# CRIMAC-WP4-Machine-learning/CRIMAC-classifiers-unet

Measured on AMD Instinct MI355X. Metric: echogram patches/sec (4ch 256x256), training step (fwd+weighted CE+bwd+SGD), higher is better.
Workload: dtype bf16; 1 GPU; BASELINE configs[1]: U-Net (depth 5, 64 filters) train step, batch 32 x 4x256x256 per GPU; global_batch=32, precision=bf16, start_filts=64, parallelism=dp1, ranks=1, launcher=single process

## Files before the change

crimac_classifiers_unet_amd/csrc/elementwise.hip:

```cpp
#include <stdarg.h>
#include <stdlib.h>

#include <mutex>

#include "common.h"
#include "bnb_sums.h"

static thread_local char g_err[512] = "";
void crimac_set_error(const char* fmt, ...) {
  va_list ap;
  va_start(ap, fmt);
  vsnprintf(g_err, sizeof(g_err), fmt, ap);
  va_end(ap);
}
extern "C" const char* crimac_last_error(void) { return g_err; }
extern "C" int crimac_version(void) { return CRIMAC_ABI_VERSION; }
extern "C" int crimac_layer_desc_size(void) { return (int)sizeof(crimac_layer_desc); }

namespace {

#ifdef CRIMAC_STREAM_FORWARD
#define CRIMAC_ROW(x, M) (x)
#else
#define CRIMAC_ROW(x, M) ((M) - 1 - (x))
#endif

constexpr int kMaxBlocks = 2048;

inline int grid_for(long work_items, int per_block) {
  long b = (work_items + per_block - 1) / per_block;
  if (b < 1) b = 1;
  if (b > kMaxBlocks) b = kMaxBlocks;
  return (int)b;
}

struct ResidentEntry { const void* fn; int dev, blocks; };
static ResidentEntry g_resident[96];
static int g_resident_n = 0;
static std::mutex g_resident_mu;
template <typename K>
inline int whole_rounds(K kernel, size_t lds, int grid, int block = 256) {
  int dev = 0;
  if (grid <= 256 || hipGetDevice(&dev) != hipSuccess) return grid;
  const void* fn = reinterpret_cast<const void*>(kernel);
  int blocks = 0;
  {
    std::lock_guard<std::mutex> lk(g_resident_mu);
    for (int i = 0; i < g_resident_n; ++i)
      if (g_resident[i].fn == fn && g_resident[i].dev == dev) blocks = g_resident[i].blocks;
    if (blocks == 0) {
      int per_cu = 0, cus = 0;
      if (hipOccupancyMaxActiveBlocksPerMultiprocessor(&per_cu, kernel, block, lds) == hipSuccess &&
          hipDeviceGetAttribute(&cus, hipDeviceAttributeMultiprocessorCount, dev) == hipSuccess && per_cu > 0 && cus > 0)
        blocks = per_cu * cus;
      else
        blocks = -1;
      if (g_resident_n < 96) g_resident[g_resident_n++] = ResidentEntry{fn, dev, blocks};
    }
  }
  return (blocks > 0 && grid > blocks) ? blocks : grid;
}

template <typename T>
__global__ void nchw_to_nhwc_kernel(const float* __restrict__ in, T* __restrict__ out, int C, long HW,
                                    long npix, long ld) {
  for (long p = blockIdx.x * (long)blockDim.x + threadIdx.x; p < npix;
       p += (long)gridDim.x * blockDim.x) {
    long b, hw;
    pix_split(p, HW, b, hw);
    const float* src = in + b * C * HW + hw;
    T* dst = out + p * ld;
    for (int c0 = 0; c0 < ld; c0 += 8) {
      float v[8];
#pragma unroll
      for (int j = 0; j < 8; ++j) v[j] = (c0 + j) < C ? src[(long)(c0 + j) * HW] : 0.f;
      store8(dst + c0, v);
// ... 73 lines not shown
      const float v = w[((long)ci * Co + co) * 4 + ab] * pf.fwd_scale;
      if (pf.interleaved) put_planes_il(v, pf.fwd_fp16, fwd_hi, r, ci, Ci);
      else put_planes(v, pf.npl, pf.fwd_fp16, fwd_hi, fwd_lo, i, n);
    }
    if (dg_hi) {
      const int co = (int)(i % Co);
      const long r = i / Co;
      const int ci = (int)(r % Ci), ab = (int)(r / Ci);
      const float v = w[((long)ci * Co + co) * 4 + ab] * pf.dg_scale;
      if (pf.interleaved) put_planes_il(v, pf.dg_fp16, dg_hi, r, co, Co);
      else put_planes(v, pf.npl, pf.dg_fp16, dg_hi, dg_lo, i, n);
    }
  }
}

__global__ void unpack_wgrad_conv_kernel(const float* __restrict__ dw, int Co, int Ci, int Ci_pad,
                                         float* __restrict__ grad) {
  const long n = (long)Co * Ci * 9;
  for (long i = blockIdx.x * (long)blockDim.x + threadIdx.x; i < n;
       i += (long)gridDim.x * blockDim.x) {
    const int t = (int)(i % 9);
    const long r = i / 9;
    const int ci = (int)(r % Ci), co = (int)(r / Ci);
    grad[i] = dw[((long)t * Co + co) * Ci_pad + ci];
  }
}

__global__ void unpack_wgrad_upconv_kernel(const float* __restrict__ dw, int Ci, int Co,
                                           float* __restrict__ grad) {
  const long n = (long)Ci * Co * 4;
  for (long i = blockIdx.x * (long)blockDim.x + threadIdx.x; i < n;
       i += (long)gridDim.x * blockDim.x) {
    const int ab = (int)(i % 4);
    const long r = i / 4;
    const int co = (int)(r % Co), ci = (int)(r / Co);
    grad[i] = dw[((long)ab * Ci + ci) * Co + co];
  }
}

template <typename T, typename ACC, int NQ, int UNR = 2, typename OP>
__device__ __forceinline__ void colreduce(long M, int C, OP op, ACC* out0, ACC* out1) {
  extern __shared__ __attribute__((aligned(16))) unsigned char smem_raw[];
  float* lds = reinterpret_cast<float*>(smem_raw);
  const int cpr = C / 8;
  const int rpi = 256 / cpr > 0 ? 256 / cpr : 1;
  for (int i = threadIdx.x; i < NQ * C; i += 256) lds[i] = 0.f;
  __syncthreads();
  const int chunk = threadIdx.x % cpr, rl = threadIdx.x / cpr;
  float s0[8], s1[8];
#pragma unroll
  for (int j = 0; j < 8; ++j) { s0[j] = 0.f; s1[j] = 0.f; }
// ... 1066 lines not shown

extern "C" int crimac_pack_upconv2x2(const float* w, int Ci, int Co, int planes, void* fwd_hi,
                                     void* fwd_lo, void* dg_hi, void* dg_lo, void* stream) {
  CRIMAC_REQUIRE(w && fwd_hi && Co > 0 && Ci > 0, "pack_upconv2x2: bad arguments");
  CRIMAC_REQUIRE(planes_arg_ok(planes) && ((planes & 15) == 1 || (planes & CRIMAC_PLANES_INTERLEAVED) || fwd_lo) &&
                     ((planes & 15) == 1 || (planes & CRIMAC_PLANES_INTERLEAVED) || !dg_hi || dg_lo),
                 "pack_upconv2x2: planes=%d needs the lo plane buffers", planes);
  const int grid = grid_for(4L * Co * Ci, 256);
  hipLaunchKernelGGL(pack_upconv_kernel, dim3(grid), dim3(256), 0, ST, w, Ci, Co, planes,
                     (unsigned short*)fwd_hi, (unsigned short*)fwd_lo, (unsigned short*)dg_hi,
                     (unsigned short*)dg_lo);
  CRIMAC_LAUNCH_CHECK();
  return CRIMAC_OK;
}

extern "C" int crimac_unpack_wgrad_conv3x3(const float* dw, int Co, int Ci, int Ci_pad, float* grad,
                                           void* stream) {
  CRIMAC_REQUIRE(dw && grad && Co > 0 && Ci > 0 && Ci_pad >= Ci, "unpack_wgrad_conv3x3: bad arguments");
  hipLaunchKernelGGL(unpack_wgrad_conv_kernel, dim3(grid_for(9L * Co * Ci, 256)), dim3(256), 0, ST, dw,
                     Co, Ci, Ci_pad, grad);
  CRIMAC_LAUNCH_CHECK();
  return CRIMAC_OK;
}

extern "C" int crimac_unpack_wgrad_upconv2x2(const float* dw, int Ci, int Co, float* grad,
                                             void* stream) {
  CRIMAC_REQUIRE(dw && grad && Co > 0 && Ci > 0, "unpack_wgrad_upconv2x2: bad arguments");
  hipLaunchKernelGGL(unpack_wgrad_upconv_kernel, dim3(grid_for(4L * Co * Ci, 256)), dim3(256), 0, ST,
                     dw, Ci, Co, grad);
  CRIMAC_LAUNCH_CHECK();
  return CRIMAC_OK;
}

static int colreduce_grid(long M, int C) {
  const int cpr = C / 8;
  const int rpi = 256 / cpr > 0 ? 256 / cpr : 1;
  return grid_for(M, rpi * 16);
}

extern "C" int crimac_colstats(int prec, const void* y, long ld, long M, int C, double* sum,
                               double* sumsq, void* stream) {
  PREC_OK("colstats");
  CRIMAC_REQUIRE(y && sum && M > 0 && C > 0 && C % 8 == 0 && C <= 2048 && ld >= C && ld % 8 == 0,
                 "colstats: bad arguments (C=%d ld=%ld)", C, ld);
  const int grid = colreduce_grid(M, C);
  const size_t lds = 2 * C * sizeof(float);
// ... 408 lines not shown
```

crimac_classifiers_unet_amd/csrc/pack.hip:

```cpp
#include "common.h"

namespace {

constexpr int kMaxLayers = 32;
constexpr int TILE = 32;

struct LayerDesc {
  const float* w;
  float* grad;
  const float* dw;
  unsigned short* fwd_hi;
  unsigned short* fwd_lo;
  unsigned short* dg_hi;
  unsigned short* dg_lo;
  int kind, Co, Ci, Ci_pad;
  int dw_splits;
  long dw_stride;
  int frag;
};

struct Table {
  LayerDesc d[kMaxLayers];
  int first[kMaxLayers + 1];
  int n;
// ... 46 lines not shown
    *reinterpret_cast<u32x4*>((k == 0 ? hi : lo + (long)(k - 1) * n) + i) = w;
  }
}

__device__ __forceinline__ void put_planes8_il(float (&v)[8], unsigned short* buf, long row, int col, int rowlen, int fp16) {
  unsigned short* dst = buf + row * 2L * rowlen + il_pos(col, rowlen);
  put_planes8(v, 2, dst, dst + il_cb(rowlen), 0, 0, fp16);
}

__device__ __forceinline__ void put_planes8_il_frag(float (&v)[8], unsigned short* buf, int t, int r, int R, int col, int rowlen,
                                                    int fp16) {
  const int c = (int)il_pos(col, rowlen);
  unsigned short* hi = buf + wfrag_index(t, r, c, R, 2 * rowlen);
  unsigned short* lo = buf + wfrag_index(t, r, c + il_cb(rowlen), R, 2 * rowlen);
  put_planes8(v, 2, hi, lo, 0, 0, fp16);
}

__global__ __launch_bounds__(256) void pack_layers_kernel(Table tb, int planes_arg) {
  __shared__ float tile[TILE][TILE * 9 + 1];
  const PlaneFmt pf = plane_fmt(planes_arg);
  const int npl = pf.npl;
  const int l = find_layer(tb, blockIdx.x);
  const LayerDesc& d = tb.d[l];
  const Geo g = geo_of(d.kind, d.Co, d.Ci, d.Ci_pad);
  const int tidx = blockIdx.x - tb.first[l];
  const int o0 = (tidx / g.tiles_inner) * TILE, i0 = (tidx % g.tiles_inner) * TILE;
  const int T = g.taps, run = TILE * T;
  const int valid = (g.inner - i0 < TILE ? (g.inner - i0 > 0 ? g.inner - i0 : 0) : TILE) * T;
  for (int ol = threadIdx.x >> 6; ol < TILE; ol += 4) {
    const float* src = d.w + ((long)(o0 + ol) * g.inner + i0) * T;
// ... 67 lines not shown
  float* base = tb.dw[l] + 4L * i;
  const long st = tb.stride[l];
  f32x4 acc = *reinterpret_cast<const f32x4*>(base + j * st);
  int k = j + kFold;
  for (; k + 3 * kFold < tb.splits[l]; k += 4 * kFold) {
    const f32x4 a = *reinterpret_cast<const f32x4*>(base + (long)k * st);
    const f32x4 b = *reinterpret_cast<const f32x4*>(base + (long)(k + kFold) * st);
    const f32x4 c = *reinterpret_cast<const f32x4*>(base + (long)(k + 2 * kFold) * st);
    const f32x4 d = *reinterpret_cast<const f32x4*>(base + (long)(k + 3 * kFold) * st);
    acc += a; acc += b; acc += c; acc += d;
  }
  for (; k < tb.splits[l]; k += kFold) acc += *reinterpret_cast<const f32x4*>(base + (long)k * st);
  *reinterpret_cast<f32x4*>(base + j * st) = acc;
}

__global__ __launch_bounds__(256) void unpack_layers_kernel(Table tb) {
  __shared__ float tile[TILE][TILE * 9 + 1];
  const int l = find_layer(tb, blockIdx.x);
  const LayerDesc& d = tb.d[l];
  const Geo g = geo_of(d.kind, d.Co, d.Ci, d.Ci_pad);
  const int tidx = blockIdx.x - tb.first[l];
  const int o0 = (tidx / g.tiles_inner) * TILE, i0 = (tidx % g.tiles_inner) * TILE;
  const int T = g.taps, run = TILE * T;
  const int nin = g.inner - i0 < TILE ? (g.inner - i0 > 0 ? g.inner - i0 : 0) : TILE;
#pragma unroll 2
  for (int idx = threadIdx.x; idx < T * TILE * TILE; idx += 256) {
    const int il = idx % TILE, ol = (idx / TILE) % TILE, t = idx / (TILE * TILE);
    if (il < nin) {
      const float* src = d.dw + ((long)t * g.outer + o0 + ol) * g.inner_pad + i0 + il;
      const int nsl = d.dw_splits < kFold ? d.dw_splits : kFold;
      float v0 = src[0], v1 = 0.f, v2 = 0.f, v3 = 0.f;
      int sp = 1;
      for (; sp + 3 < nsl; sp += 4) {
        const float a = src[(long)sp * d.dw_stride], b = src[(long)(sp + 1) * d.dw_stride];
        const float c = src[(long)(sp + 2) * d.dw_stride], e = src[(long)(sp + 3) * d.dw_stride];
        v0 += a; v1 += b; v2 += c; v3 += e;
      }
      for (; sp < nsl; ++sp) v0 += src[(long)sp * d.dw_stride];
      tile[ol][il * T + t] = (v0 + v1) + (v2 + v3);
    }
  }
  __syncthreads();
  const int valid = nin * T;
  for (int ol = threadIdx.x >> 6; ol < TILE; ol += 4) {
    float* dst = d.grad + ((long)(o0 + ol) * g.inner + i0) * T;
    for (int r = threadIdx.x & 63; r < valid; r += 64) dst[r] = tile[ol][r];
  }
}

struct HostDesc {
  const float* w;
  float* grad;
  const float* dw;
  void *fwd_hi, *fwd_lo, *dg_hi, *dg_lo;
  int kind, Co, Ci, Ci_pad;
  int dw_splits;
  long dw_stride;
};

int run_layers(const HostDesc* descs, int n, int mode, int planes_arg, hipStream_t st) {
  const int planes = planes_arg & 15;
  for (int base = 0; base < n; base += kMaxLayers) {
    Table tb;
    tb.n = n - base < kMaxLayers ? n - base : kMaxLayers;
    int total = 0;
    for (int i = 0; i < tb.n; ++i) {
      HostDesc h = descs[base + i];
      const int frag = ((h.kind & CRIMAC_LAYER_FWD_FRAG) ? 1 : 0) | ((h.kind & CRIMAC_LAYER_DG_FRAG) ? 2 : 0);
      CRIMAC_REQUIRE((h.kind & ~(3 | CRIMAC_LAYER_FWD_FRAG | CRIMAC_LAYER_DG_FRAG)) == 0 && (h.kind & 3) != 3 && h.Co > 0 &&
                     h.Ci > 0, "layer %d: bad kind/shape", base + i);
      h.kind &= 3;
      if (frag && mode == 0) {
        const bool ilv = (planes_arg & CRIMAC_PLANES_INTERLEAVED) != 0;
        const int kq = ilv ? 32 : 64;
        CRIMAC_REQUIRE(h.kind == 0 && (planes == 1 || ilv),
                       "layer %d: fragment-major planes are a single-plane 16-bit or interleaved-pair Conv2d layout", base + i);
        CRIMAC_REQUIRE(!(frag & 1) || (h.Co % 32 == 0 && h.Ci_pad % kq == 0), "layer %d: fragment-major forward plane needs "
                       "Co %% 32 == 0 and Ci_pad %% %d == 0 (Co=%d Ci_pad=%d)", base + i, kq, h.Co, h.Ci_pad);
        CRIMAC_REQUIRE(!(frag & 2) || (h.dg_hi && h.Ci % 32 == 0 && h.Co % kq == 0 && h.Ci_pad == h.Ci),
                       "layer %d: fragment-major input-gradient plane needs Ci %% 32 == 0 and Co %% %d == 0", base + i, kq);
      }
      CRIMAC_REQUIRE(h.Co % TILE == 0 && (h.kind == 0 || h.Ci % TILE == 0),
                     "layer %d: Co (and the transposed convolution's Ci) must be multiples of %d", base + i, TILE);
      CRIMAC_REQUIRE(h.kind == 1 || (h.Ci_pad >= h.Ci && h.Ci_pad % 2 == 0), "layer %d: bad Ci_pad", base + i);
      if (mode == 0) {
        const bool il = (planes_arg & CRIMAC_PLANES_INTERLEAVED) != 0;
        CRIMAC_REQUIRE(h.w && h.fwd_hi && (planes == 1 || il || h.fwd_lo) && (planes == 1 || il || !h.dg_hi || h.dg_lo),
                       "layer %d: missing weight / plane pointers", base + i);
        CRIMAC_REQUIRE(!il || h.kind == 1 || h.Ci_pad % 8 == 0, "layer %d: interleaved planes need Ci_pad %% 8 == 0", base + i);
        CRIMAC_REQUIRE(h.kind != 2 || planes == 1 || (h.fwd_lo && (!h.dg_hi || h.dg_lo)),
                       "layer %d: a 1x1 layer's low planes are separate buffers in every multi-plane mode", base + i);
        CRIMAC_REQUIRE(h.kind == 1 || !h.dg_hi || h.Ci_pad == h.Ci, "layer %d: dgrad planes need Ci_pad == Ci",
                       base + i);
      } else {
        CRIMAC_REQUIRE(h.dw && h.grad, "layer %d: missing dw / grad pointers", base + i);
      }
      LayerDesc& d = tb.d[i];
      d.w = h.w; d.grad = h.grad; d.dw = h.dw;
      d.fwd_hi = (unsigned short*)h.fwd_hi; d.fwd_lo = (unsigned short*)h.fwd_lo;
      d.dg_hi = (unsigned short*)h.dg_hi; d.dg_lo = (unsigned short*)h.dg_lo;
      d.kind = h.kind; d.Co = h.Co; d.Ci = h.Ci; d.Ci_pad = h.kind == 0 ? h.Ci_pad : h.Ci;
      d.dw_splits = h.dw_splits; d.dw_stride = h.dw_stride;
      d.frag = mode == 0 ? frag : 0;
      if (mode == 1)
        CRIMAC_REQUIRE(h.dw_splits <= 1 || h.dw_stride >= (long)taps_of(h.kind) * h.Co * (h.kind == 0 ? h.Ci_pad : h.Ci),
                       "layer %d: dw_stride smaller than one packed gradient", base + i);
      const Geo g = geo_of(d.kind, d.Co, d.Ci, d.Ci_pad);
      tb.first[i] = total;
      total += (g.outer / TILE) * g.tiles_inner;
    }
    tb.first[tb.n] = total;
    if (total == 0) continue;
    if (mode == 1) {
      FoldTable ft;
      ft.n = 0;
      int fb = 0;
      for (int i = 0; i < tb.n; ++i) {
        const LayerDesc& d = tb.d[i];
        if (d.dw_splits <= kFold) continue;
        const long nfl = (long)taps_of(d.kind) * d.Co * d.Ci_pad;
        CRIMAC_REQUIRE(nfl % 4 == 0 && d.dw_stride % 4 == 0 && ((uintptr_t)d.dw % 16 == 0),
                       "layer %d: partial slabs must be 16-byte aligned", base + i);
        ft.dw[ft.n] = const_cast<float*>(d.dw); ft.stride[ft.n] = d.dw_stride; ft.splits[ft.n] = d.dw_splits;
        ft.n4[ft.n] = (int)(nfl / 4); ft.first[ft.n] = fb;
        fb += (int)((nfl / 4 + 255) / 256);
        ++ft.n;
      }
      if (ft.n) {
        ft.first[ft.n] = fb;
        hipLaunchKernelGGL(fold_slabs_kernel, dim3(fb, kFold), dim3(256), 0, st, ft);
        CRIMAC_LAUNCH_CHECK();
      }
    }
    if (mode == 0) hipLaunchKernelGGL(pack_layers_kernel, dim3(total), dim3(256), 0, st, tb, planes_arg);
    else hipLaunchKernelGGL(unpack_layers_kernel, dim3(total), dim3(256), 0, st, tb);
    CRIMAC_LAUNCH_CHECK();
  }
  return CRIMAC_OK;
}

}

extern "C" int crimac_pack_layers(const crimac_layer_desc* descs, int n_layers, int planes, void* stream) {
  CRIMAC_REQUIRE(descs && n_layers > 0 && planes_arg_ok(planes), "pack_layers: bad arguments (planes=%d)", planes);
  return run_layers(reinterpret_cast<const HostDesc*>(descs), n_layers, 0, planes, (hipStream_t)stream);
}

extern "C" int crimac_unpack_wgrad_layers(const crimac_layer_desc* descs, int n_layers, void* stream) {
  CRIMAC_REQUIRE(descs && n_layers > 0, "unpack_wgrad_layers: bad arguments");
  return run_layers(reinterpret_cast<const HostDesc*>(descs), n_layers, 1, 1, (hipStream_t)stream);
}
```

crimac_classifiers_unet_amd/engine.py:

```python
from __future__ import annotations

import contextlib
import ctypes as C
import os

import torch

from . import hip
from .hip import Act, call, ptr


def _on_device(fn):
    import functools

    @functools.wraps(fn)
    def wrapped(self, *a, **kw):
        if getattr(self, "device", None) is None:
            self.bind()
        dev = self.device
        if dev is None or dev.type != "cuda":
            return fn(self, *a, **kw)
        with torch.cuda.device(dev):
            return fn(self, *a, **kw)
    return wrapped

BN_EPS = 1e-5
BN_MOMENTUM = 0.1
CIN_PAD = 16
NARROW_WIDTHS = (8, 16, 32)
STAT_REPLICAS = 64


def _align(n, a=64):
    return (n + a - 1) // a * a


class _ConvBlock:

    def __init__(self, conv_key, bn_key, cin, cout, cin_pad=None):
        self.conv_key, self.bn_key = conv_key, bn_key
        self.cin, self.cout = cin, cout
        self.cin_pad = cin_pad or cin
        self.idx = None
        self.narrow = False


class _UpConv:

    def __init__(self, key, cin, cout, mode="transpose"):
# ... 107 lines not shown
        if dev.type != "cuda":
            raise hip.HipLibraryError(
                "UNet_Baseline (MI355X build) must live on a GPU: call .to('cuda'); "
                "there is no CPU fallback for the hot path")
        ok = self.device == dev and getattr(self, "flat_p", None) is not None
        if ok:
            base = self.flat_p.data_ptr()
            for name, p in params:
                off, n, _ = self.layout[name]
                if p.data_ptr() != base + 4 * off or p.dtype != torch.float32:
                    ok = False
                    break
        if ok:
            return
        self.device = dev
        self.layout, off = {}, 0
        for name, p in params:
            self.layout[name] = (off, p.numel(), tuple(p.shape))
            off += _align(p.numel())
        self.n_flat = off
        flat_p = torch.zeros(off, dtype=torch.float32, device=dev)
        self.flat_g = torch.zeros(off, dtype=torch.float32, device=dev)
        self.flat_v = torch.zeros(off, dtype=torch.float32, device=dev)
        with torch.no_grad():
            for name, p in params:
                o, n, shp = self.layout[name]
                flat_p[o:o + n].copy_(p.detach().reshape(-1).float())
                p.data = flat_p[o:o + n].view(shp)
                p.grad = self.flat_g[o:o + n].view(shp)
        self.flat_p = flat_p
        self.P = {name: p for name, p in params}
        self.G = {name: self.flat_g[o:o + n].view(shp) for name, (o, n, shp) in self.layout.items()}
        self.Bf = dict(self.module.named_buffers())
        self._alloc_static()
        self._train_pack_dirty = self._eval_pack_dirty = True
        self._bufs = {}

    def _alloc_static(self):
        dev = self.device
        i16 = torch.int16
        self._ltab = None
        self.pk = self.pk_main = {}
        self.pk_eval = {}
        self.dw_plan = None
        self.dw_off = {}
        self.dw_packed = None
        il = self.is_hp
        m_hi = 2 if il else 1
        for b in self.blocks:
            if b.narrow:
                self.pk[b.conv_key] = {"narrow": True, "key": b.conv_key, "w_cin": b.cin, "frag_ok": (False, False),
                                       "fwd_frag": False, "dg_frag": False}
                self.pk_eval[b.conv_key] = {"narrow": True, "key": b.conv_key, "w_cin": b.cin, "fwd_frag": False,
                                            "bias": torch.empty(b.cout, dtype=torch.float32, device=dev),
                                            "scale": torch.empty(b.cout, dtype=torch.float32, device=dev)}
                continue
            n_f = 9 * b.cout * b.cin_pad
            n_lo = max(self.planes - 1, 1)
            has_dg = b.cin_pad == b.cin
            self.pk[b.conv_key] = {
                "fwd_hi": torch.empty(m_hi * n_f, dtype=i16, device=dev),
# ... 115 lines not shown
            for b in self.enc[i]:
                add(b.conv_key, 0, b.cout, b.cin_pad, 9 * b.cout * b.cin_pad, h, w)
        for j in range(D - 1):
            L = D - 2 - j
            h, w, _ = geo[L]
            for b in self.dec[j]:
                add(b.conv_key, 0, b.cout, b.cin_pad, 9 * b.cout * b.cin_pad, h, w)
            u = self.ups[j]
            hp, wp, _ = geo[L + 1]
            if u.up1x1:
                add(u.key, None, u.cout, u.cin, u.cout * u.cin, hp, wp)
            else:
                add(u.key, 1, u.cin, u.cout, 4 * u.cin * u.cout, hp, wp)
        self.dw_off = off
        self.dw_packed = torch.zeros(tot, dtype=torch.float32, device=self.device)
        self.dw_plan = (B, H, W, self.use_wgrad_partials)
        self._ltab = None

    def _dw(self, key):
        o, sp, stride = self.dw_off[key]
        return self.dw_packed[o:o + sp * stride], sp, stride

    def mark_dirty(self):
        self._train_pack_dirty = self._eval_pack_dirty = True
        self._packed_groups = set()
        for f in self._followers:
            f._train_pack_dirty = f._eval_pack_dirty = True
            f._packed_groups = set()

    def _check_versions(self):
        v = sum(p._version for p in self.P.values()) + sum(b._version for b in self.Bf.values())
        if v != self._versions:
            self._versions = v
            self.mark_dirty()

    def _layer_table(self):
# ... 180 lines not shown
                                          self.wgrad_target_blocks)
        self._on_side(lambda: call(name, *args, flops=flops, mfmas=hip.MFMAS_PER_PRODUCT[prec]))

    def _join_wgrad(self):
        if self._side is not None:
            for side in self._side:
                torch.cuda.current_stream().wait_stream(side)

    def _unpack_group(self, gi, on_ready=None, rng=None):
        self._flush_wgrad_group()
        arr, bounds = self._layer_table()
        first, n = bounds[gi]

        def unpack():
            if n:
                call("crimac_unpack_wgrad_layers", C.byref(arr, first * C.sizeof(hip.LayerDesc)), n)
            self._unpack_narrow(gi)

        side = self._single_side()
        if side is None:
            self._join_wgrad()
            unpack()
            if on_ready is not None:
                on_ready(*rng)
            return
        with self._fork_side(side):
            unpack()
            if on_ready is not None and self.exchange_on_side:
                on_ready(*rng)
            done = torch.cuda.Event()
            done.record()
            self._unpacked[gi] = done
        if on_ready is not None and not self.exchange_on_side:
            torch.cuda.current_stream().wait_stream(side)
            on_ready(*rng)

    def _unpack_narrow(self, gi):
        for l in self._narrow_groups[gi]:
            if isinstance(l, _UpConv):
                call("crimac_unpack_wgrad_upconv2x2", ptr(self._dw(l.key)[0]), l.cin, l.cout, ptr(self.G[l.key + ".weight"]))
            else:
                call("crimac_unpack_wgrad_conv3x3", ptr(self._dw(l.conv_key)[0]), l.cout, l.cin, l.cin_pad,
                     ptr(self.G[l.conv_key + ".weight"]))

    def _pack_ups(self):
        if self.up_mode == "upsample":
            arr, _ = self._layer_table()
            sub = (hip.LayerDesc * len(self.ups))(*[d for d in arr if (d.kind & 3) == hip.LAYER_CONV1X1])
            call("crimac_pack_layers", C.byref(sub), len(sub), self._fwd_planes_arg())
            return
        for u in self.ups:
            if u.narrow:
                continue
            pk = self.pk[u.key]
            call("crimac_pack_upconv2x2", ptr(self.P[u.key + ".weight"]), u.cin, u.cout, self.planes_arg,
                 ptr(pk["fwd_hi"]), ptr(pk["fwd_lo"]), ptr(pk["dg_hi"]), ptr(pk["dg_lo"]))

    def _pack_eval(self):
# ... 554 lines not shown

    @_on_device
    def backward(self, dlogits, on_ready=None, before_join=None):
        ranges = self.grad_ranges() if on_ready is not None else None
        s = self.saved
        if s is None:
            raise RuntimeError("backward() needs a preceding train-mode forward()")
        B, H, W = s["B"], s["H"], s["W"]
        geo = self._geom(B, H, W)
        D = self.depth
        self._skip_done = {}
        self._unpacked = {}
        self._wg_pending, self._wg_launches = [], 0
        self._dup16 = {}
        self._plan_dw(B, H, W)
        self.flat_g.zero_()
        if not self.use_wgrad_partials:
            self.dw_packed.zero_()
        self.stat[2:].zero_()
        self.bias_scr.zero_()
        dlogits = dlogits.contiguous().float()
        head_in = s["head_in"]
        h, w, M = geo[0]
        d_cur = Act(self._buf("g.head", (M, self.sf)), self.sf)
        head_fused = self.fuse_bn_bwd and D >= 2
        if head_in is None and not head_fused:
            raise RuntimeError("head input was not materialised (fuse_head_bn) but the fused BatchNorm sums are off")
        bnb = self._bnb_args(self.dec[D - 2][1], s[f"d{D - 2}"][4] if head_fused else None)
        x_args = (head_in.p if head_in is not None else None, head_in.ld if head_in is not None else 0)
        if self.lmi:
            pre = "post_processing_weights.main."
            call("crimac_head_meta_bwd", self.prec, ptr(dlogits), *x_args, ptr(self.P["conv_final.weight"]), d_cur.p,
                 d_cur.ld, ptr(self.G["conv_final.weight"]), ptr(self.G["conv_final.bias"]), ptr(s["meta"]),
# ... 56 lines not shown
                     *self._bnb_args(b2, y2 if self.fuse_bn_bwd else None))
            da1 = Act(self._buf(f"g.e{i}.a1", (M, c)), c)
            fused = self._block_bwd(f"g.e{i}.2", b2, da2, y2, a1, B, h, w, M, da1, next_bn=(b1, y1),
                                    reduce_done=(self.fuse_bn_bwd and i != D - 1) or (i == D - 1 and cur_done),
                                    unpool_src=unpool_src)
            d_pool = Act(self._buf(f"g.e{i}.xin", (M, b1.cin)), b1.cin) if i > 0 else None
            self._block_bwd(f"g.e{i}.1", b1, da1, y1, x_in, B, h, w, M, d_pool, reduce_done=fused)
            g = self._enc_group(i)
            if i == 0 or self._enc_group(i - 1) != g:
                self._unpack_group(g, on_ready, ranges[g] if ranges else None)
        self._flush_wgrad_group()
        self._wg_pending = None
        if before_join is not None:
            before_join()
        self._join_wgrad()

    def _labels(self, labels):
        if not labels.is_cuda:
            raise hip.HipLibraryError("labels are not on a GPU")
        if labels.dtype not in (torch.int16, torch.int32, torch.int64):
            labels = labels.long()
        return labels.contiguous()

    @_on_device
    def ce_forward(self, logits, labels, class_w, ignore_index=-100, sums=None):
        labels = self._labels(labels)
        B, nc, H, W = logits.shape
        if tuple(labels.shape) != (B, H, W):
            raise ValueError(f"labels {tuple(labels.shape)} do not match logits {tuple(logits.shape)}")
        if sums is None:
# ... 218 lines not shown
```

crimac_classifiers_unet_amd/hip.py:

```python
from __future__ import annotations

import ctypes as C
import os
import re

import torch

from . import build as _build

PREC_BF16 = 0
PREC_F32X3 = 1
PREC_F32X6 = 2
PREC_FP16 = 3
PREC_F32H3 = 4
PREC_H3P = 5
PREC_H3F_BWD = 6
PREC_NAMES = {"bf16": PREC_BF16, "f32x3": PREC_F32X3, "f32x6": PREC_F32X6, "fp16": PREC_FP16, "f32h3": PREC_F32H3,
              "h3p": PREC_H3P, "h3f": PREC_H3P}
MFMAS_PER_PRODUCT = {PREC_BF16: 1, PREC_FP16: 1, PREC_F32X3: 3, PREC_F32H3: 3, PREC_H3P: 3, PREC_F32X6: 6, PREC_H3F_BWD: 1}
PREC_PLANES = {PREC_BF16: 1, PREC_F32X3: 2, PREC_F32X6: 3, PREC_FP16: 1, PREC_F32H3: 2, PREC_H3P: 2}
PLANES_FP16 = 1 | 16 | 32
PLANES_F32H3 = 2 | 16 | (8 << 8)
PLANES_FWD_FRAG = 65536
PLANES_INTERLEAVED = 64
PLANES_H3P = 2 | 16 | 32 | PLANES_INTERLEAVED | 128 | (8 << 8)
PREC_PLANES_ARG = {PREC_BF16: 1, PREC_F32X3: 2, PREC_F32X6: 3, PREC_FP16: PLANES_FP16, PREC_F32H3: PLANES_F32H3,
                   PREC_H3P: PLANES_H3P}
EPI_RELU, EPI_OUT_PLANES, EPI_CIN4 = 1, 2, 4
EPI_WFRAG = 16
EPI_WROWS = 32
NARROW_DGRAD = 64
LAYER_FWD_FRAG, LAYER_DG_FRAG = 16, 32
LAYER_CONV3X3, LAYER_UPCONV2X2, LAYER_CONV1X1 = 0, 1, 2
PREC_BACKWARD = {PREC_F32H3: PREC_F32X3}
PREC_16BIT = (PREC_BF16, PREC_FP16)


class HipLibraryError(RuntimeError):
    pass


_SCALARS = {"int": C.c_int, "long": C.c_long, "long long": C.c_longlong, "unsigned int": C.c_uint,
            "unsigned long long": C.c_ulonglong, "float": C.c_float, "double": C.c_double}
_KEYWORDS = {"const", "void", "char", "short", "signed", "struct", *" ".join(_SCALARS).split()}


def _declarator(decl: str, where: str):
    toks = decl.replace("*", " * ").split()
# ... 205 lines not shown
```

include/crimac_unet_hip.h:

```cpp
#ifndef CRIMAC_UNET_HIP_H_
#define CRIMAC_UNET_HIP_H_

#ifdef __cplusplus
extern "C" {
#endif

#define CRIMAC_OK 0
#define CRIMAC_ERR_INVALID (-22)
#define CRIMAC_ERR_LAUNCH (-5)

#define CRIMAC_PREC_BF16 0
#define CRIMAC_PREC_F32X3 1
#define CRIMAC_PREC_F32X6 2
#define CRIMAC_PREC_FP16 3
#define CRIMAC_PREC_F32H3 4
#define CRIMAC_PREC_H3P 5
#define CRIMAC_PREC_MAX 5
#define CRIMAC_PREC_H3F_BWD 6
#define CRIMAC_F32H3_WSHIFT 8
#define CRIMAC_PLANES_FWD_FP16 16
#define CRIMAC_PLANES_DG_FP16 32
#define CRIMAC_PLANES_FP16 (1 | CRIMAC_PLANES_FWD_FP16 | CRIMAC_PLANES_DG_FP16)
#define CRIMAC_PLANES_F32H3 (2 | CRIMAC_PLANES_FWD_FP16 | (CRIMAC_F32H3_WSHIFT << 8))
#define CRIMAC_PLANES_INTERLEAVED 64
// ... 71 lines not shown
int crimac_up2x_adjoint(int prec, const void* dy, long dy_ld, int B, int H, int W, int C, void* dz, long dz_ld,
                        void* stream);
int crimac_conv1x1_dgrad(int prec, const void* dz, long dz_ld, int B, int H, int W, int Cout, int Cin, const void* w_dg_hi,
                         const void* w_dg_lo, void* dx, long dx_ld, void* stream);
int crimac_conv1x1_wgrad(int prec, const void* dz, long dz_ld, int Cout, const void* x, long x_ld, int Cin, long M,
                         float* dw, void* stream);



int crimac_pack_conv3x3(const float* w, int Co, int Ci, int Ci_pad, const float* scale, int planes,
                        void* fwd_hi, void* fwd_lo, void* dg_hi, void* dg_lo, void* stream);
int crimac_pack_upconv2x2(const float* w, int Ci, int Co, int planes, void* fwd_hi, void* fwd_lo,
                          void* dg_hi, void* dg_lo, void* stream);
int crimac_unpack_wgrad_conv3x3(const float* dw, int Co, int Ci, int Ci_pad, float* grad, void* stream);
int crimac_unpack_wgrad_upconv2x2(const float* dw, int Ci, int Co, float* grad, void* stream);

typedef struct crimac_layer_desc {
  const float* w;
  float* grad;
  const float* dw;
  void* fwd_hi;
  void* fwd_lo;
  void* dg_hi;
  void* dg_lo;
  int kind;
  int Co, Ci, Ci_pad;
  int dw_splits;
  long dw_stride;
} crimac_layer_desc;
#define CRIMAC_LAYER_FWD_FRAG 16
#define CRIMAC_LAYER_DG_FRAG 32
int crimac_pack_layers(const crimac_layer_desc* descs, int n_layers, int planes, void* stream);
int crimac_unpack_wgrad_layers(const crimac_layer_desc* descs, int n_layers, void* stream);


int crimac_nchw_to_nhwc(int prec, const float* in, void* out, int B, int C, int H, int W, long ld,
                        void* stream);


int crimac_colstats(int prec, const void* y, long ld, long M, int C, double* sum, double* sumsq,
                    void* stream);
int crimac_colsum_f32(int prec, const void* y, long ld, long M, int C, float* sum, void* stream);
int crimac_sum_replicas(const double* src, int replicas, long stride, int n, double* dst_f64,
                        float* dst_f32, const double* src_b, double* dst_b_f64, void* stream);
int crimac_bn_finalize(const double* sum, const double* sumsq, int replicas, long M, int C, const float* gamma,
                       const float* beta, float eps, float momentum, float* running_mean,
                       float* running_var, long long* num_batches_tracked, float* mean,
                       float* invstd, float* scale, float* shift, void* stream);
// ... 226 lines not shown
```

Baseline: 2927 patches/s.

## Zero packed wgrad buffers during unpack and skip full gradient memsets

The wgrad unpack kernels can now zero the packed dw buffer behind themselves. This replaces the full dw_packed.zero_() each step, which is only redone when a step left the buffer dirty. The full flat_g memset becomes a ranged zero covering only the gradient regions the unpack table does not overwrite. The table unpack kernel also becomes a persistent, prefetching, vectorised-store loop over tiles, sorted by tap count. This removes two large memset passes per step, at the cost of more intricate invariants: the buffers must start clean, and the scheme is restricted to dw_splits<=1.

Result: no change. 2940 patches/s, median of 6 (+0.5%).

```diff
diff --git a/crimac_classifiers_unet_amd/csrc/elementwise.hip b/crimac_classifiers_unet_amd/csrc/elementwise.hip
--- a/crimac_classifiers_unet_amd/csrc/elementwise.hip
+++ b/crimac_classifiers_unet_amd/csrc/elementwise.hip
@@ -5,6 +5,7 @@
 
 #include "common.h"
 #include "bnb_sums.h"
+#include "whole_rounds.h"
 
 static thread_local char g_err[512] = "";
 void crimac_set_error(const char* fmt, ...) {
@@ -34,32 +35,6 @@
   return (int)b;
 }
 
-struct ResidentEntry { const void* fn; int dev, blocks; };
-static ResidentEntry g_resident[96];
-static int g_resident_n = 0;
-static std::mutex g_resident_mu;
-template <typename K>
-inline int whole_rounds(K kernel, size_t lds, int grid, int block = 256) {
-  int dev = 0;
-  if (grid <= 256 || hipGetDevice(&dev) != hipSuccess) return grid;
-  const void* fn = reinterpret_cast<const void*>(kernel);
-  int blocks = 0;
-  {
-    std::lock_guard<std::mutex> lk(g_resident_mu);
-    for (int i = 0; i < g_resident_n; ++i)
-      if (g_resident[i].fn == fn && g_resident[i].dev == dev) blocks = g_resident[i].blocks;
-    if (blocks == 0) {
-      int per_cu = 0, cus = 0;
-      if (hipOccupancyMaxActiveBlocksPerMultiprocessor(&per_cu, kernel, block, lds) == hipSuccess &&
-          hipDeviceGetAttribute(&cus, hipDeviceAttributeMultiprocessorCount, dev) == hipSuccess && per_cu > 0 && cus > 0)
-        blocks = per_cu * cus;
-      else
-        blocks = -1;
-      if (g_resident_n < 96) g_resident[g_resident_n++] = ResidentEntry{fn, dev, blocks};
-    }
-  }
-  return (blocks > 0 && grid > blocks) ? blocks : grid;
-}
 
 template <typename T>
 __global__ void nchw_to_nhwc_kernel(const float* __restrict__ in, T* __restrict__ out, int C, long HW,
@@ -163,27 +138,37 @@
   }
 }
 
-__global__ void unpack_wgrad_conv_kernel(const float* __restrict__ dw, int Co, int Ci, int Ci_pad,
-                                         float* __restrict__ grad) {
+__global__ void unpack_wgrad_conv_kernel(float* __restrict__ dw, int Co, int Ci, int Ci_pad,
+                                         float* __restrict__ grad, int zero) {
   const long n = (long)Co * Ci * 9;
   for (long i = blockIdx.x * (long)blockDim.x + threadIdx.x; i < n;
        i += (long)gridDim.x * blockDim.x) {
     const int t = (int)(i % 9);
     const long r = i / 9;
     const int ci = (int)(r % Ci), co = (int)(r / Ci);
-    grad[i] = dw[((long)t * Co + co) * Ci_pad + ci];
-  }
-}
-
-__global__ void unpack_wgrad_upconv_kernel(const float* __restrict__ dw, int Ci, int Co,
-                                           float* __restrict__ grad) {
+    float* src = dw + ((long)t * Co + co) * Ci_pad + ci;
+    grad[i] = *src;
+    if (zero) *src = 0.f;
+  }
+  if (zero && Ci_pad > Ci) {
+    const int npad = Ci_pad - Ci;
+    const long m = 9L * Co * npad;
+    for (long i = blockIdx.x * (long)blockDim.x + threadIdx.x; i < m; i += (long)gridDim.x * blockDim.x)
+      dw[(i / npad) * Ci_pad + Ci + (int)(i % npad)] = 0.f;
+  }
+}
+
+__global__ void unpack_wgrad_upconv_kernel(float* __restrict__ dw, int Ci, int Co,
+                                           float* __restrict__ grad, int zero) {
   const long n = (long)Ci * Co * 4;
   for (long i = blockIdx.x * (long)blockDim.x + threadIdx.x; i < n;
        i += (long)gridDim.x * blockDim.x) {
     const int ab = (int)(i % 4);
     const long r = i / 4;
     const int co = (int)(r % Co), ci = (int)(r / Co);
-    grad[i] = dw[((long)ab * Ci + ci) * Co + co];
+    float* src = dw + ((long)ab * Ci + ci) * Co + co;
+    grad[i] = *src;
+    if (zero) *src = 0.f;
   }
 }
 
@@ -1280,22 +1265,34 @@
   return CRIMAC_OK;
 }
 
+extern "C" int crimac_unpack_wgrad_conv3x3_flags(float* dw, int Co, int Ci, int Ci_pad, float* grad, int flags,
+                                                 void* stream) {
+  CRIMAC_REQUIRE(dw && grad && Co > 0 && Ci > 0 && Ci_pad >= Ci && (flags & ~CRIMAC_UNPACK_ZERO_BEHIND) == 0,
+                 "unpack_wgrad_conv3x3: bad arguments");
+  hipLaunchKernelGGL(unpack_wgrad_conv_kernel, dim3(grid_for(9L * Co * Ci, 256)), dim3(256), 0, ST, dw,
+                     Co, Ci, Ci_pad, grad, (flags & CRIMAC_UNPACK_ZERO_BEHIND) ? 1 : 0);
+  CRIMAC_LAUNCH_CHECK();
+  return CRIMAC_OK;
+}
+
 extern "C" int crimac_unpack_wgrad_conv3x3(const float* dw, int Co, int Ci, int Ci_pad, float* grad,
                                            void* stream) {
-  CRIMAC_REQUIRE(dw && grad && Co > 0 && Ci > 0 && Ci_pad >= Ci, "unpack_wgrad_conv3x3: bad arguments");
-  hipLaunchKernelGGL(unpack_wgrad_conv_kernel, dim3(grid_for(9L * Co * Ci, 256)), dim3(256), 0, ST, dw,
-                     Co, Ci, Ci_pad, grad);
+  return crimac_unpack_wgrad_conv3x3_flags(const_cast<float*>(dw), Co, Ci, Ci_pad, grad, 0, stream);
+}
+
+extern "C" int crimac_unpack_wgrad_upconv2x2_flags(float* dw, int Ci, int Co, float* grad, int flags,
+                                                   void* stream) {
+  CRIMAC_REQUIRE(dw && grad && Co > 0 && Ci > 0 && (flags & ~CRIMAC_UNPACK_ZERO_BEHIND) == 0,
+                 "unpack_wgrad_upconv2x2: bad arguments");
+  hipLaunchKernelGGL(unpack_wgrad_upconv_kernel, dim3(grid_for(4L * Co * Ci, 256)), dim3(256), 0, ST,
+                     dw, Ci, Co, grad, (flags & CRIMAC_UNPACK_ZERO_BEHIND) ? 1 : 0);
   CRIMAC_LAUNCH_CHECK();
   return CRIMAC_OK;
 }
 
 extern "C" int crimac_unpack_wgrad_upconv2x2(const float* dw, int Ci, int Co, float* grad,
                                              void* stream) {
-  CRIMAC_REQUIRE(dw && grad && Co > 0 && Ci > 0, "unpack_wgrad_upconv2x2: bad arguments");
-  hipLaunchKernelGGL(unpack_wgrad_upconv_kernel, dim3(grid_for(4L * Co * Ci, 256)), dim3(256), 0, ST,
-                     dw, Ci, Co, grad);
-  CRIMAC_LAUNCH_CHECK();
-  return CRIMAC_OK;
+  return crimac_unpack_wgrad_upconv2x2_flags(const_cast<float*>(dw), Ci, Co, grad, 0, stream);
 }
 
 static int colreduce_grid(long M, int C) {
diff --git a/crimac_classifiers_unet_amd/csrc/pack.hip b/crimac_classifiers_unet_amd/csrc/pack.hip
--- a/crimac_classifiers_unet_amd/csrc/pack.hip
+++ b/crimac_classifiers_unet_amd/csrc/pack.hip
@@ -1,4 +1,5 @@
 #include "common.h"
+#include "whole_rounds.h"
 
 namespace {
 
@@ -84,6 +85,42 @@
   unsigned short* hi = buf + wfrag_index(t, r, c, R, 2 * rowlen);
   unsigned short* lo = buf + wfrag_index(t, r, c + il_cb(rowlen), R, 2 * rowlen);
   put_planes8(v, 2, hi, lo, 0, 0, fp16);
+}
+
+struct TileAt {
+  int l, o0, i0;
+};
+__device__ __forceinline__ TileAt tile_at(const Table& tb, int item) {
+  TileAt a;
+  a.l = find_layer(tb, item);
+  const LayerDesc& d = tb.d[a.l];
+  const int tiles_inner = ((d.kind == 1 ? d.Co : d.Ci_pad) + TILE - 1) / TILE;
+  const int tidx = item - tb.first[a.l];
+  a.o0 = (tidx / tiles_inner) * TILE;
+  a.i0 = (tidx % tiles_inner) * TILE;
+  return a;
+}
+
+template <int T>
+__device__ __forceinline__ void rows_store(float* grad, int inner, int o0, int i0, const float (&tile)[TILE][TILE * 9 + 1]) {
+#pragma unroll 3
+  for (int j = 0; j < T; ++j) {
+    const int k = threadIdx.x + 256 * j, row = k / (8 * T), c4 = k % (8 * T);
+    f32x4 v;
+#pragma unroll
+    for (int e = 0; e < 4; ++e) v[e] = tile[row][4 * c4 + e];
+    *(reinterpret_cast<f32x4*>(grad + ((long)(o0 + row) * inner + i0) * T) + c4) = v;
+  }
+}
+#define CRIMAC_FOR_TAPS(T, ...)          \
+  do {                                   \
+    if ((T) == 9) { __VA_ARGS__(9); }    \
+    else if ((T) == 4) { __VA_ARGS__(4); } \
+    else { __VA_ARGS__(1); }             \
+  } while (0)
+
+__device__ __forceinline__ bool rows_aligned(const void* p, const Geo& g, int i0) {
+  return g.inner - i0 >= TILE && (g.inner * g.taps) % 4 == 0 && (reinterpret_cast<uintptr_t>(p) & 15) == 0;
 }
 
 __global__ __launch_bounds__(256) void pack_layers_kernel(Table tb, int planes_arg) {
@@ -181,38 +218,112 @@
   *reinterpret_cast<f32x4*>(base + j * st) = acc;
 }
 
-__global__ __launch_bounds__(256) void unpack_layers_kernel(Table tb) {
+__global__ __launch_bounds__(256, 4) void unpack_layers_kernel(Table tb, int zero_behind) {
   __shared__ float tile[TILE][TILE * 9 + 1];
-  const int l = find_layer(tb, blockIdx.x);
-  const LayerDesc& d = tb.d[l];
-  const Geo g = geo_of(d.kind, d.Co, d.Ci, d.Ci_pad);
-  const int tidx = blockIdx.x - tb.first[l];
-  const int o0 = (tidx / g.tiles_inner) * TILE, i0 = (tidx % g.tiles_inner) * TILE;
-  const int T = g.taps, run = TILE * T;
-  const int nin = g.inner - i0 < TILE ? (g.inner - i0 > 0 ? g.inner - i0 : 0) : TILE;
+  const int total = tb.first[tb.n];
+  int item = blockIdx.x;
+  if (item >= total) return;
+  f32x4 regs[9];
+  TileAt at = tile_at(tb, item);
+  bool pre = false;
+#define CRIMAC_PACKED_ROW(dd, gg, aa, t)                                                                              \
+  (reinterpret_cast<f32x4*>(const_cast<float*>((dd).dw) + ((long)(t) * (gg).outer + (aa).o0 + (threadIdx.x >> 3)) * (gg).inner_pad + \
+                            (aa).i0) + (threadIdx.x & 7))
+#define CRIMAC_PACKED_OK(dd, gg, aa)                                                                                  \
+  ((dd).dw_splits <= 1 && (gg).inner - (aa).i0 >= TILE && (gg).inner_pad % 4 == 0 && (reinterpret_cast<uintptr_t>((dd).dw) & 15) == 0)
+  {
+    const LayerDesc& d = tb.d[at.l];
+    const Geo g = geo_of(d.kind, d.Co, d.Ci, d.Ci_pad);
+    if (CRIMAC_PACKED_OK(d, g, at)) {
+#pragma unroll
+      for (int t = 0; t < 9; ++t)
+        if (t < g.taps) regs[t] = *CRIMAC_PACKED_ROW(d, g, at, t);
+      pre = true;
+    }
+  }
+  while (true) {
+    const LayerDesc& d = tb.d[at.l];
+    const Geo g = geo_of(d.kind, d.Co, d.Ci, d.Ci_pad);
+    const int o0 = at.o0, i0 = at.i0;
+    const int T = g.taps;
+    const int nin = g.inner - i0 < TILE ? (g.inner - i0 > 0 ? g.inner - i0 : 0) : TILE;
+    if (pre) {
+      const int ol = threadIdx.x >> 3, il = (threadIdx.x & 7) * 4;
+#pragma unroll
+      for (int t = 0; t < 9; ++t)
+        if (t < T) {
+#pragma unroll
+          for (int e = 0; e < 4; ++e) tile[ol][(il + e) * T + t] = regs[t][e];
+        }
+      if (zero_behind) {
+#pragma unroll
+        for (int t = 0; t < 9; ++t)
+          if (t < T) *CRIMAC_PACKED_ROW(d, g, at, t) = f32x4{0.f, 0.f, 0.f, 0.f};
+      }
+    } else {
 #pragma unroll 2
-  for (int idx = threadIdx.x; idx < T * TILE * TILE; idx += 256) {
-    const int il = idx % TILE, ol = (idx / TILE) % TILE, t = idx / (TILE * TILE);
-    if (il < nin) {
-      const float* src = d.dw + ((long)t * g.outer + o0 + ol) * g.inner_pad + i0 + il;
-      const int nsl = d.dw_splits < kFold ? d.dw_splits : kFold;
-      float v0 = src[0], v1 = 0.f, v2 = 0.f, v3 = 0.f;
-      int sp = 1;
-      for (; sp + 3 < nsl; sp += 4) {
-        const float a = src[(long)sp * d.dw_stride], b = src[(long)(sp + 1) * d.dw_stride];
-        const float c = src[(long)(sp + 2) * d.dw_stride], e = src[(long)(sp + 3) * d.dw_stride];
-        v0 += a; v1 += b; v2 += c; v3 += e;
-      }
-      for (; sp < nsl; ++sp) v0 += src[(long)sp * d.dw_stride];
-      tile[ol][il * T + t] = (v0 + v1) + (v2 + v3);
-    }
-  }
-  __syncthreads();
-  const int valid = nin * T;
-  for (int ol = threadIdx.x >> 6; ol < TILE; ol += 4) {
-    float* dst = d.grad + ((long)(o0 + ol) * g.inner + i0) * T;
-    for (int r = threadIdx.x & 63; r < valid; r += 64) dst[r] = tile[ol][r];
-  }
+      for (int idx = threadIdx.x; idx < T * TILE * TILE; idx += 256) {
+        const int il = idx % TILE, ol = (idx / TILE) % TILE, t = idx / (TILE * TILE);
+        float* src = const_cast<float*>(d.dw) + ((long)t * g.outer + o0 + ol) * g.inner_pad + i0 + il;
+        if (il < nin) {
+          const int nsl = d.dw_splits < kFold ? d.dw_splits : kFold;
+          float v0 = src[0], v1 = 0.f, v2 = 0.f, v3 = 0.f;
+          int sp = 1;
+          for (; sp + 3 < nsl; sp += 4) {
+            const float a = src[(long)sp * d.dw_stride], b = src[(long)(sp + 1) * d.dw_stride];
+            const float c = src[(long)(sp + 2) * d.dw_stride], e = src[(long)(sp + 3) * d.dw_stride];
+            v0 += a; v1 += b; v2 += c; v3 += e;
+          }
+          for (; sp < nsl; ++sp) v0 += src[(long)sp * d.dw_stride];
+          tile[ol][il * T + t] = (v0 + v1) + (v2 + v3);
+        }
+        if (zero_behind && i0 + il < g.inner_pad) src[0] = 0.f;
+      }
+    }
+    __syncthreads();
+    const int next = item + gridDim.x;
+    TileAt nat = at;
+    bool npre = false;
+    if (next < total) {
+      nat = tile_at(tb, next);
+      const LayerDesc& nd = tb.d[nat.l];
+      const Geo ng = geo_of(nd.kind, nd.Co, nd.Ci, nd.Ci_pad);
+      if (CRIMAC_PACKED_OK(nd, ng, nat)) {
+#pragma unroll
+        for (int t = 0; t < 9; ++t)
+          if (t < ng.taps) regs[t] = *CRIMAC_PACKED_ROW(nd, ng, nat, t);
+        npre = true;
+      }
+    }
+    if (rows_aligned(d.grad, g, i0)) {
+#define CRIMAC_STORE(TT) rows_store<TT>(d.grad, g.inner, o0, i0, tile)
+      CRIMAC_FOR_TAPS(T, CRIMAC_STORE);
+    } else {
+      const int valid = nin * T;
+      for (int ol = threadIdx.x >> 6; ol < TILE; ol += 4) {
+        float* dst = d.grad + ((long)(o0 + ol) * g.inner + i0) * T;
+        for (int r = threadIdx.x & 63; r < valid; r += 64) dst[r] = tile[ol][r];
+      }
+    }
+    if (next >= total) break;
+    __syncthreads();
+    item = next; at = nat; pre = npre;
+  }
+}
+
+constexpr int kMaxRanges = 64;
+struct RangeTable {
+  long first[kMaxRanges], count[kMaxRanges];
+  int block0[kMaxRanges + 1];
+  int n;
+};
+__global__ __launch_bounds__(256) void zero_ranges_kernel(float* base, RangeTable rt) {
+  int r = 0;
+  while (r + 1 < rt.n && (int)blockIdx.x >= rt.block0[r + 1]) ++r;
+  const long lo = (long)(blockIdx.x - rt.block0[r]) * 4096;
+  const long hi = lo + 4096 < rt.count[r] ? lo + 4096 : rt.count[r];
+  float* p = base + rt.first[r];
+  for (long i = lo + threadIdx.x; i < hi; i += 256) p[i] = 0.f;
 }
 
 struct HostDesc {
@@ -225,13 +336,25 @@
   long dw_stride;
 };
 
-int run_layers(const HostDesc* descs, int n, int mode, int planes_arg, hipStream_t st) {
+template <typename K>
+int persistent_grid(K kernel, int total) {
+  const int resident = whole_rounds(kernel, 0, total);
+  const int per_wg = (total + resident - 1) / resident;
+  return (total + per_wg - 1) / per_wg;
+}
+
+int run_layers(const HostDesc* descs, int n, int mode, int planes_arg, hipStream_t st, int flags = 0) {
   const int planes = planes_arg & 15;
   for (int base = 0; base < n; base += kMaxLayers) {
     Table tb;
     tb.n = n - base < kMaxLayers ? n - base : kMaxLayers;
     int total = 0;
-    for (int i = 0; i < tb.n; ++i) {
+    int order[kMaxLayers], no = 0;
+    for (int taps = 9; taps >= 1; --taps)
+      for (int i = 0; i < tb.n; ++i)
+        if (taps_of(descs[base + i].kind & 3) == taps) order[no++] = i;
+    for (int s = 0; s < tb.n; ++s) {
+      const int i = order[s];
       HostDesc h = descs[base + i];
       const int frag = ((h.kind & CRIMAC_LAYER_FWD_FRAG) ? 1 : 0) | ((h.kind & CRIMAC_LAYER_DG_FRAG) ? 2 : 0);
       CRIMAC_REQUIRE((h.kind & ~(3 | CRIMAC_LAYER_FWD_FRAG | CRIMAC_LAYER_DG_FRAG)) == 0 && (h.kind & 3) != 3 && h.Co > 0 &&
@@ -261,8 +384,10 @@
                        base + i);
       } else {
         CRIMAC_REQUIRE(h.dw && h.grad, "layer %d: missing dw / grad pointers", base + i);
-      }
-      LayerDesc& d = tb.d[i];
+        CRIMAC_REQUIRE(!(flags & CRIMAC_UNPACK_ZERO_BEHIND) || h.dw_splits <= 1,
+                       "layer %d: CRIMAC_UNPACK_ZERO_BEHIND is for finished sums (dw_splits <= 1), not for partial slabs", base + i);
+      }
+      LayerDesc& d = tb.d[s];
       d.w = h.w; d.grad = h.grad; d.dw = h.dw;
       d.fwd_hi = (unsigned short*)h.fwd_hi; d.fwd_lo = (unsigned short*)h.fwd_lo;
       d.dg_hi = (unsigned short*)h.dg_hi; d.dg_lo = (unsigned short*)h.dg_lo;
@@ -273,7 +398,7 @@
         CRIMAC_REQUIRE(h.dw_splits <= 1 || h.dw_stride >= (long)taps_of(h.kind) * h.Co * (h.kind == 0 ? h.Ci_pad : h.Ci),
                        "layer %d: dw_stride smaller than one packed gradient", base + i);
       const Geo g = geo_of(d.kind, d.Co, d.Ci, d.Ci_pad);
-      tb.first[i] = total;
+      tb.first[s] = total;
       total += (g.outer / TILE) * g.tiles_inner;
     }
     tb.first[tb.n] = total;
@@ -299,8 +424,11 @@
         CRIMAC_LAUNCH_CHECK();
       }
     }
-    if (mode == 0) hipLaunchKernelGGL(pack_layers_kernel, dim3(total), dim3(256), 0, st, tb, planes_arg);
-    else hipLaunchKernelGGL(unpack_layers_kernel, dim3(total), dim3(256), 0, st, tb);
+    if (mode == 0)
+      hipLaunchKernelGGL(pack_layers_kernel, dim3(total), dim3(256), 0, st, tb, planes_arg);
+    else
+      hipLaunchKernelGGL(unpack_layers_kernel, dim3(persistent_grid(unpack_layers_kernel, total)), dim3(256), 0, st, tb,
+                         (flags & CRIMAC_UNPACK_ZERO_BEHIND) ? 1 : 0);
     CRIMAC_LAUNCH_CHECK();
   }
   return CRIMAC_OK;
@@ -317,3 +445,30 @@
   CRIMAC_REQUIRE(descs && n_layers > 0, "unpack_wgrad_layers: bad arguments");
   return run_layers(reinterpret_cast<const HostDesc*>(descs), n_layers, 1, 1, (hipStream_t)stream);
 }
+
+extern "C" int crimac_unpack_wgrad_layers_flags(const crimac_layer_desc* descs, int n_layers, int flags, void* stream) {
+  CRIMAC_REQUIRE(descs && n_layers > 0 && (flags & ~CRIMAC_UNPACK_ZERO_BEHIND) == 0, "unpack_wgrad_layers_flags: bad arguments");
+  return run_layers(reinterpret_cast<const HostDesc*>(descs), n_layers, 1, 1, (hipStream_t)stream, flags);
+}
+
+extern "C" int crimac_zero_ranges(float* base, const long* ranges, int n_ranges, void* stream) {
+  CRIMAC_REQUIRE(base && ranges && n_ranges > 0, "zero_ranges: bad arguments");
+  for (int r0 = 0; r0 < n_ranges; r0 += kMaxRanges) {
+    RangeTable rt;
+    rt.n = n_ranges - r0 < kMaxRanges ? n_ranges - r0 : kMaxRanges;
+    long blocks = 0;
+    for (int r = 0; r < rt.n; ++r) {
+      rt.first[r] = ranges[2 * (r0 + r)];
+      rt.count[r] = ranges[2 * (r0 + r) + 1];
+      CRIMAC_REQUIRE(rt.first[r] >= 0 && rt.count[r] >= 0, "zero_ranges: range %d is negative", r0 + r);
+      rt.block0[r] = (int)blocks;
+      blocks += (rt.count[r] + 4095) / 4096;
+      CRIMAC_REQUIRE(blocks < (1L << 30), "zero_ranges: too many elements");
+    }
+    rt.block0[rt.n] = (int)blocks;
+    if (blocks == 0) continue;
+    hipLaunchKernelGGL(zero_ranges_kernel, dim3((unsigned)blocks), dim3(256), 0, (hipStream_t)stream, base, rt);
+    CRIMAC_LAUNCH_CHECK();
+  }
+  return CRIMAC_OK;
+}
diff --git a/crimac_classifiers_unet_amd/csrc/whole_rounds.h b/crimac_classifiers_unet_amd/csrc/whole_rounds.h
--- /dev/null
+++ b/crimac_classifiers_unet_amd/csrc/whole_rounds.h
@@ -0,0 +1,41 @@
+#pragma once
+#include <hip/hip_runtime.h>
+
+#include <mutex>
+
+namespace {
+
+struct ResidentEntry { const void* fn; int dev, blocks; };
+static ResidentEntry g_resident[96];
+static int g_resident_n = 0;
+static std::mutex g_resident_mu;
+
+template <typename K>
+inline int resident_blocks(K kernel, size_t lds, int block = 256) {
+  int dev = 0;
+  if (hipGetDevice(&dev) != hipSuccess) return 0;
+  const void* fn = reinterpret_cast<const void*>(kernel);
+  int blocks = 0;
+  std::lock_guard<std::mutex> lk(g_resident_mu);
+  for (int i = 0; i < g_resident_n; ++i)
+    if (g_resident[i].fn == fn && g_resident[i].dev == dev) blocks = g_resident[i].blocks;
+  if (blocks == 0) {
+    int per_cu = 0, cus = 0;
+    if (hipOccupancyMaxActiveBlocksPerMultiprocessor(&per_cu, kernel, block, lds) == hipSuccess &&
+        hipDeviceGetAttribute(&cus, hipDeviceAttributeMultiprocessorCount, dev) == hipSuccess && per_cu > 0 && cus > 0)
+      blocks = per_cu * cus;
+    else
+      blocks = -1;
+    if (g_resident_n < 96) g_resident[g_resident_n++] = ResidentEntry{fn, dev, blocks};
+  }
+  return blocks > 0 ? blocks : 0;
+}
+
+template <typename K>
+inline int whole_rounds(K kernel, size_t lds, int grid, int block = 256) {
+  if (grid <= 256) return grid;
+  const int blocks = resident_blocks(kernel, lds, block);
+  return (blocks > 0 && grid > blocks) ? blocks : grid;
+}
+
+}
diff --git a/crimac_classifiers_unet_amd/engine.py b/crimac_classifiers_unet_amd/engine.py
--- a/crimac_classifiers_unet_amd/engine.py
+++ b/crimac_classifiers_unet_amd/engine.py
@@ -33,6 +33,25 @@
 
 def _align(n, a=64):
     return (n + a - 1) // a * a
+
+
+def flat_layout(named_params):
+    layout, off = {}, 0
+    for name, p in named_params:
+        layout[name] = (off, p.numel(), tuple(p.shape))
+        off += _align(p.numel())
+    return layout, off
+
+
+def uncovered_ranges(layout, n_flat, covered):
+    out, pos = [], 0
+    for o, n in sorted((layout[k][0], layout[k][1]) for k in covered):
+        if o > pos:
+            out.append((pos, o - pos))
+        pos = max(pos, o + n)
+    if pos < n_flat:
+        out.append((pos, n_flat - pos))
+    return out
 
 
 class _ConvBlock:
@@ -170,10 +189,7 @@
         if ok:
             return
         self.device = dev
-        self.layout, off = {}, 0
-        for name, p in params:
-            self.layout[name] = (off, p.numel(), tuple(p.shape))
-            off += _align(p.numel())
+        self.layout, off = flat_layout(params)
         self.n_flat = off
         flat_p = torch.zeros(off, dtype=torch.float32, device=dev)
         self.flat_g = torch.zeros(off, dtype=torch.float32, device=dev)
@@ -201,6 +217,8 @@
         self.dw_plan = None
         self.dw_off = {}
         self.dw_packed = None
+        self._dw_dirty = False
+        self._gzero = None
         il = self.is_hp
         m_hi = 2 if il else 1
         for b in self.blocks:
@@ -346,12 +364,25 @@
                 add(u.key, 1, u.cin, u.cout, 4 * u.cin * u.cout, hp, wp)
         self.dw_off = off
         self.dw_packed = torch.zeros(tot, dtype=torch.float32, device=self.device)
+        self._dw_dirty = False
         self.dw_plan = (B, H, W, self.use_wgrad_partials)
         self._ltab = None
 
     def _dw(self, key):
         o, sp, stride = self.dw_off[key]
         return self.dw_packed[o:o + sp * stride], sp, stride
+
+    def table_weight_keys(self):
+        return ([b.conv_key + ".weight" for b in self.blocks if not b.narrow]
+                + [u.key + ".weight" for u in self.ups if not u.narrow])
+
+    def _zero_unwritten_grads(self):
+        if self._gzero is None:
+            rngs = uncovered_ranges(self.layout, self.n_flat, self.table_weight_keys())
+            self._gzero = ((C.c_long * (2 * len(rngs)))(*[v for r in rngs for v in r]), len(rngs))
+        arr, n = self._gzero
+        if n:
+            call("crimac_zero_ranges", ptr(self.flat_g), arr, n)
 
     def mark_dirty(self):
         self._train_pack_dirty = self._eval_pack_dirty = True
@@ -562,7 +593,7 @@
 
         def unpack():
             if n:
-                call("crimac_unpack_wgrad_layers", C.byref(arr, first * C.sizeof(hip.LayerDesc)), n)
+                call("crimac_unpack_wgrad_layers_flags", C.byref(arr, first * C.sizeof(hip.LayerDesc)), n, self._unpack_flags())
             self._unpack_narrow(gi)
 
         side = self._single_side()
@@ -583,13 +614,17 @@
             torch.cuda.current_stream().wait_stream(side)
             on_ready(*rng)
 
+    def _unpack_flags(self):
+        return 0 if self.use_wgrad_partials else hip.UNPACK_ZERO_BEHIND
+
     def _unpack_narrow(self, gi):
         for l in self._narrow_groups[gi]:
             if isinstance(l, _UpConv):
-                call("crimac_unpack_wgrad_upconv2x2", ptr(self._dw(l.key)[0]), l.cin, l.cout, ptr(self.G[l.key + ".weight"]))
+                call("crimac_unpack_wgrad_upconv2x2_flags", ptr(self._dw(l.key)[0]), l.cin, l.cout,
+                     ptr(self.G[l.key + ".weight"]), self._unpack_flags())
             else:
-                call("crimac_unpack_wgrad_conv3x3", ptr(self._dw(l.conv_key)[0]), l.cout, l.cin, l.cin_pad,
-                     ptr(self.G[l.conv_key + ".weight"]))
+                call("crimac_unpack_wgrad_conv3x3_flags", ptr(self._dw(l.conv_key)[0]), l.cout, l.cin, l.cin_pad,
+                     ptr(self.G[l.conv_key + ".weight"]), self._unpack_flags())
 
     def _pack_ups(self):
         if self.up_mode == "upsample":
@@ -1174,9 +1209,10 @@
         self._wg_pending, self._wg_launches = [], 0
         self._dup16 = {}
         self._plan_dw(B, H, W)
-        self.flat_g.zero_()
-        if not self.use_wgrad_partials:
+        self._zero_unwritten_grads()
+        if self._dw_dirty and not self.use_wgrad_partials:
             self.dw_packed.zero_()
+        self._dw_dirty = True
         self.stat[2:].zero_()
         self.bias_scr.zero_()
         dlogits = dlogits.contiguous().float()
@@ -1263,6 +1299,7 @@
         if before_join is not None:
             before_join()
         self._join_wgrad()
+        self._dw_dirty = False
 
     def _labels(self, labels):
         if not labels.is_cuda:
diff --git a/crimac_classifiers_unet_amd/hip.py b/crimac_classifiers_unet_amd/hip.py
--- a/crimac_classifiers_unet_amd/hip.py
+++ b/crimac_classifiers_unet_amd/hip.py
@@ -32,6 +32,7 @@
 NARROW_DGRAD = 64
 LAYER_FWD_FRAG, LAYER_DG_FRAG = 16, 32
 LAYER_CONV3X3, LAYER_UPCONV2X2, LAYER_CONV1X1 = 0, 1, 2
+UNPACK_ZERO_BEHIND = 1
 PREC_BACKWARD = {PREC_F32H3: PREC_F32X3}
 PREC_16BIT = (PREC_BF16, PREC_FP16)
 
diff --git a/include/crimac_unet_hip.h b/include/crimac_unet_hip.h
--- a/include/crimac_unet_hip.h
+++ b/include/crimac_unet_hip.h
@@ -109,6 +109,9 @@
                           void* dg_hi, void* dg_lo, void* stream);
 int crimac_unpack_wgrad_conv3x3(const float* dw, int Co, int Ci, int Ci_pad, float* grad, void* stream);
 int crimac_unpack_wgrad_upconv2x2(const float* dw, int Ci, int Co, float* grad, void* stream);
+#define CRIMAC_UNPACK_ZERO_BEHIND 1
+int crimac_unpack_wgrad_conv3x3_flags(float* dw, int Co, int Ci, int Ci_pad, float* grad, int flags, void* stream);
+int crimac_unpack_wgrad_upconv2x2_flags(float* dw, int Ci, int Co, float* grad, int flags, void* stream);
 
 typedef struct crimac_layer_desc {
   const float* w;
@@ -127,6 +130,8 @@
 #define CRIMAC_LAYER_DG_FRAG 32
 int crimac_pack_layers(const crimac_layer_desc* descs, int n_layers, int planes, void* stream);
 int crimac_unpack_wgrad_layers(const crimac_layer_desc* descs, int n_layers, void* stream);
+int crimac_unpack_wgrad_layers_flags(const crimac_layer_desc* descs, int n_layers, int flags, void* stream);
+int crimac_zero_ranges(float* base, const long* ranges, int n_ranges, void* stream);
 
 
 int crimac_nchw_to_nhwc(int prec, const float* in, void* out, int B, int C, int H, int W, long ld,
```
